# HKUST-Aerial-Robotics/Omni-swarm

Measured on AMD Instinct MI355X. Metric: keyframes/sec (4x fisheye 600x480) + p50 loop-match ms @ 100k-frame DB, higher is better.
Workload: dtype f16

## Files before the change

### omni-swarm_amd/csrc/config.h

```cpp
#pragma once
#include "common.h"

namespace omni {

enum CfgId {
    CFG_CONV_V1 = 0, CFG_RS_TRN, CFG_DET16, CFG_SP_SPARSE_DESC, CFG_SP_SPARSE_DA, CFG_SP_FUSED_CAND, CFG_SP_SPLIT_DB, CFG_SP_MASK_SKIP, CFG_SP_MASK_SKIP_SPLIT, CFG_SPLIT_FUSE1A, CFG_SPLIT_WINO,
    CFG_SPLIT_TRN, CFG_CONV_XCD, CFG_SP_PROFILE_MASK, CFG_PP_U8, CFG_PP_TRACE, CFG_PP_DBG, CFG_RS_TRACE, CFG_SPLIT_TRACE, CFG_SPLIT_DBG, CFG_WINO_TRACE, CFG_ROCTX,
    CFG_VLAD_BIG, CFG_VLAD_STEM_FUSE, CFG_VLAD_UNFUSED, CFG_VLAD_MFMA, CFG_VLAD_SBLOCK, CFG_VLAD_MBLOCK_PX, CFG_VLAD_MFMA_PX, CFG_VLAD_FC_MFMA, CFG_VLAD_MBLOCK_CPW,
    CFG_VLAD_SB_LDSPAD, CFG_VLAD_SB_PERSIST, CFG_VLAD_SB_TRACE, CFG_VLAD_SB_DBG, CFG_VLAD_MASK_SKIP,
    CFG_SCAN_ROWS_MIN, CFG_MQ_ROT, CFG_MQ_MIN, CFG_INDEX_MIRROR, CFG_INDEX_MIRROR_MIN_ROWS, CFG_INDEX_CERT_FAIL,
    CFG_GEOMETRY_THREADS, CFG_MESSAGE_THREADS, CFG_GEOMETRY_ASYNC, CFG_DETECTOR_ASYNC, CFG_PIPELINE_ONE_STREAM, CFG_PIPELINE_FIFO, CFG_PIPELINE_UNIT_PLAN,
    CFG_HW_QUEUES,
    CFG_RCCL_LIB,
    CFG_COUNT
};
enum CfgClass {
    CFG_VARIANT = 0,
    CFG_TUNING = 1,
    CFG_DEBUG = 2,
    CFG_TEST = 3,
    CFG_STRING = 4
};
struct CfgOption { const char* env; int def, lo, hi; int cls; const char* doc; };
extern const CfgOption kCfgOptions[CFG_COUNT];

struct Config {
    int v[CFG_COUNT];
    int operator[](CfgId i) const { return v[i]; }
};
int config_resolve(Config* out);
const Config& config_process();
int config_option_now(CfgId i);

}
```

### omni-swarm_amd/csrc/config.hip

```cpp
#include "config.h"

#include <atomic>
#include <cerrno>
#include <climits>
#include <cstdlib>

namespace omni {

const CfgOption kCfgOptions[CFG_COUNT] = {
    {"OMNI_CONV_V1", 0, 0, 3, CFG_VARIANT, "fp16 3x3 layers: 0 = production (conv1a fused into the ping-pong conv1b, register-stationary cin=128); 1 = generic kernel, 2 = persistent LDS-DMA kernel, "
                                           "3 = ping-pong without the conv1a fusion -- 1-3 exist only in the test build of the library (lib_test/)"},
    {"OMNI_RS_TRN", -1, -1, 1, CFG_VARIANT, "register-stationary kernel of the unpooled cin=128 fp16 layers: tile orientation, -1 = the one with fewer tiles, 0 = plain, 1 = transposed"},
    {"OMNI_DET16", 1, 0, 1, CFG_VARIANT, "detector head of the fp16 and OMNI_PREC_SPLIT paths on v_mfma_f32_32x32x16_f16 with split (hi, lo) operands (0: the exact-f32 MFMA kernel)"},
    {"OMNI_SP_SPARSE_DESC", 1, 0, 1, CFG_VARIANT, "convDb + descriptor norm only at the cells around the key points (0: dense descriptor map)"},
    {"OMNI_SP_SPARSE_DA", 1, 0, 1, CFG_VARIANT, "convDa only at those cells too (fp16 and OMNI_PREC_SPLIT; 0: dense convDa)"},
    {"OMNI_SP_FUSED_CAND", 1, 0, 1, CFG_VARIANT, "getKeyPoints' threshold inside the detector head's epilogue + window masks from the candidate list (0: sp_cand_kernel re-reads the heat map)"},
    {"OMNI_SP_SPLIT_DB", 1, 0, 1, CFG_VARIANT, "OMNI_PREC_SPLIT: convDb + descriptor norm at the key points' cells with split (hi, lo) operands on the fp16 matrix cores (0: exact-f32 MFMA convolution)"},
    {"OMNI_SP_MASK_SKIP", 1, 0, 1, CFG_VARIANT, "fp16: the tiles inside the constant region of the fisheye mask are left out of the tile walk (0: every tile)"},
    {"OMNI_SP_MASK_SKIP_SPLIT", 1, 0, 1, CFG_VARIANT, "the same for OMNI_PREC_SPLIT"},
    {"OMNI_SPLIT_FUSE1A", 1, 0, 1, CFG_VARIANT, "OMNI_PREC_SPLIT: conv1a built inside the conv1b kernel from the u8 image (0: separate exact-f32 conv1a pass)"},
    {"OMNI_SPLIT_WINO", 7, 0, 15, CFG_VARIANT, "OMNI_PREC_SPLIT: the cin = 64 layers as Winograd F(2x2,3x3) kernels with split operands (conv_wino.hip), bit 0 = conv1b (with the conv1a "
                                                "fusion), 1 = conv2a, 2 = conv2b, 3 = conv3a (off by default: same time as the direct kernel, profiles/r06g); 0: the direct kernels of conv_split.hip"},
    {"OMNI_SPLIT_TRN", -1, -1, 1, CFG_VARIANT, "OMNI_PREC_SPLIT cin=128 kernel: tile orientation, as OMNI_RS_TRN"},
    {"OMNI_CONV_XCD", 1, 0, 1, CFG_VARIANT, "persistent convolution kernels derive (cout group, tile walk) from an XCD-aware block id: the cout groups of a pixel tile and its neighbours "
                                           "share one L2 (0: plain blockIdx; process-wide, same results either way)"},
    {"OMNI_SP_PROFILE_MASK", 0, 0, 1, CFG_TUNING, "omni_sp_profile times the stages with the fisheye mask on (what the key-frame pipeline runs)"},
    {"OMNI_PP_U8", 1, 0, 1, CFG_VARIANT, "fp16 conv1a inside conv1b's kernel: matrix-core operands straight from the image bytes (0: through the 256-entry u8 -> (hi, lo) table in LDS)"},
    {"OMNI_PP_TRACE", 0, 0, 1, CFG_DEBUG, "s_memtime trace of the ping-pong conv kernel on stderr"},
    {"OMNI_PP_DBG", 0, 0, 255, CFG_DEBUG, "ping-pong conv kernel timing ablations (WRONG results)"},
    {"OMNI_RS_TRACE", 0, 0, 1, CFG_DEBUG, "s_memtime trace of the register-stationary kernel"},
    {"OMNI_SPLIT_TRACE", 0, 0, 1, CFG_DEBUG, "s_memtime trace of the split-precision kernel"},
    {"OMNI_SPLIT_DBG", 0, 0, 3, CFG_DEBUG, "split-precision kernel timing ablations: 1 = no stores, 2 = every DMA reads tile 0 (WRONG results)"},
    {"OMNI_WINO_TRACE", 0, 0, 1, CFG_DEBUG, "s_memtime trace of the Winograd split kernel"},
    {"OMNI_ROCTX", 0, 0, 1, CFG_DEBUG, "roctx ranges around upload / SuperPoint / MobileNetVLAD / post-processing / BF match / index add + search / exchange and the host loop's "
                                      "stages (rocprofv3 --marker-trace; the library is resolved by dlopen)"},
    {"OMNI_VLAD_BIG", 0, 0, 128, CFG_TUNING, "64 / 128: the 64- / 128-pixel tiles of the unfused block kernel (measured slower at 600x480)"},
    {"OMNI_VLAD_STEM_FUSE", 1, 0, 1, CFG_VARIANT, "stem + block 0 in one kernel (0: two kernels)"},
    {"OMNI_VLAD_UNFUSED", 0, 0, 1, CFG_VARIANT, "1: every block as expand / depthwise / project launches"},
    {"OMNI_VLAD_MFMA", 1, 0, 1, CFG_VARIANT, "late blocks' 1x1 convolutions on the matrix cores"},
    {"OMNI_VLAD_SBLOCK", 1, 0, 1, CFG_VARIANT, "fused split-fp16 block kernel (vlad_s.hip)"},
    {"OMNI_VLAD_MBLOCK_PX", 2048, 0, 1 << 24, CFG_TUNING, "fused matrix-core block kernel for blocks of at most this many input pixels per image (0 disables)"},
    {"OMNI_VLAD_MFMA_PX", 0, 0, 1 << 24, CFG_TUNING, "> 0: matrix-core 1x1 convolutions for blocks of at most this many input pixels per image (default 2048)"},
    {"OMNI_VLAD_FC_MFMA", 1, 0, 1, CFG_VARIANT, "the final FC on the matrix cores (0: VALU kernel)"},
    {"OMNI_VLAD_MBLOCK_CPW", 0, 0, 64, CFG_TUNING, "hidden-layer split of the matrix-core block kernel: chunks per workgroup (0 = no split; measured: does not pay)"},
    {"OMNI_VLAD_SB_LDSPAD", 0, 0, 160 * 1024, CFG_DEBUG, "extra LDS bytes per workgroup of the split block kernel (occupancy A/B)"},
    {"OMNI_VLAD_SB_PERSIST", 1, 0, 16, CFG_VARIANT, "split block kernel: 0 = one tile per workgroup, N >= 1 = N x (CUs x resident workgroups) persistent workgroups"},
    {"OMNI_VLAD_SB_TRACE", 0, 0, 1, CFG_DEBUG, "s_memtime trace of the split block kernel"},
    {"OMNI_VLAD_SB_DBG", 0, 0, 255, CFG_DEBUG, "split block kernel timing ablations (WRONG results)"},
    {"OMNI_VLAD_MASK_SKIP", 1, 0, 1, CFG_VARIANT, "fisheye-masked passes leave the tiles of the first blocks that lie in the constant region of the mask out of the tile walk "
                                                  "(bit-identical; 0: the dense pass)"},
    {"OMNI_SCAN_ROWS_MIN", 4, 1, 1 << 20, CFG_TUNING, "fp32 scan: from this many queries on, the rows-stationary kernel"},
    {"OMNI_MQ_ROT", 1, 0, 1, CFG_VARIANT, "matrix-core multi-query scan: rotated query fragments"},
    {"OMNI_MQ_MIN", 4, 0, 1 << 20, CFG_TUNING, "queries from which an fp16 shard is searched on the matrix cores (1 = always, 0 = never)"},
    {"OMNI_INDEX_MIRROR", 1, 0, 1, CFG_VARIANT, "fp32 index: fp16 mirror + certificate for batched searches (0: exact scans only)"},
    {"OMNI_INDEX_MIRROR_MIN_ROWS", 32768, 0, INT_MAX, CFG_TUNING, "the mirror is used from this many rows on"},
    {"OMNI_INDEX_CERT_FAIL", 0, 0, 1, CFG_TEST, "1: every certificate fails (exercises the exact fallback)"},
    {"OMNI_GEOMETRY_THREADS", -1, -1, 1024, CFG_TUNING, "threads of the geometric-verification pool (-1: min(16, cores / 2); 0: inline)"},
    {"OMNI_MESSAGE_THREADS", 3, 0, 64, CFG_TUNING, "helper threads that fill a unit's key-frame messages (key points, descriptors, lifted points: ~75 KB per image, first-touch page "
                                                  "faults included) next to the calling thread while the unit's detector step runs on the GPU (0: inline)"},
    {"OMNI_GEOMETRY_ASYNC", 1, 0, 1, CFG_VARIANT, "a micro-batch's geometry tasks run while the next unit is waited for (0: drained at once)"},
    {"OMNI_DETECTOR_ASYNC", 1, 0, 1, CFG_VARIANT, "a micro-batch's detector step (appends, searches) is enqueued and collected one unit later (0: the host waits for it on the spot)"},
    {"OMNI_PIPELINE_ONE_STREAM", 0, 0, 1, CFG_VARIANT, "a unit's MobileNetVLAD launches behind its SuperPoint launches on one stream (0: next to them on a second stream)"},
    {"OMNI_PIPELINE_FIFO", -1, -1, 2, CFG_VARIANT, "units in flight run oldest first: a unit's SuperPoint stream (1) / both its streams (2) start behind the convolution stack of the unit "
                                                   "enqueued before it; 0: the units' kernels take turns; -1: by measurement -- 1 for the fp32-class precisions, whose time is all "
                                                   "CU-filling convolutions (+2-4 %), and for an fp16 run() of no more units than lanes (all in flight at once: +13 % at 3 units), 0 for fp16 otherwise, whose small-grid "
                                                   "tails the next units' kernels fill (-5 % when chained)"},
    {"OMNI_PIPELINE_UNIT_PLAN", 1, 0, 2, CFG_VARIANT, "KeyframePipeline::run on host blocks, a run that is not a whole number of micro-batches: 1 = units of equal size (20 key frames = "
                                                       "7 + 7 + 6), 2 = the same behind half a unit, 0 = the blocks' own cut (8 + 8 + 4)"},
    {"OMNI_HW_QUEUES", 8, 0, 64, CFG_TUNING, "hardware queues asked of the HIP runtime when the library is loaded (GPU_MAX_HW_QUEUES, unless already set): the pipeline's five "
                                            "streams must not share one; 0 = the runtime's default of 4"},
    {"OMNI_RCCL_LIB", 0, 0, 0, CFG_STRING, "path of the RCCL library omni_shard dlopens (default: librccl.so next to torch, then the loader's search path)"},
};

static int parse_one(const CfgOption& o, int* out, bool* bad) {
    *out = o.def; *bad = false;
    if (o.cls == CFG_STRING) return 0;
    const char* e = getenv(o.env);
    if (!e || !e[0]) return 0;
    errno = 0;
    char* end = nullptr;
    const long v = strtol(e, &end, 10);
    if (errno || end == e || *end != '\0' || v < o.lo || v > o.hi) { *bad = true; return 0; }
    *out = (int)v;
    return 1;
}

int config_resolve(Config* out) {
    for (int i = 0; i < CFG_COUNT; ++i) {
        bool bad;
        parse_one(kCfgOptions[i], &out->v[i], &bad);
        OMNI_REQUIRE(!bad, OMNI_ERR_INVALID, "%s=%s: expected an integer in [%d, %d] (%s)", kCfgOptions[i].env, getenv(kCfgOptions[i].env), kCfgOptions[i].lo, kCfgOptions[i].hi,
                     kCfgOptions[i].doc);
    }
    return OMNI_OK;
}

static bool is_process_wide(int i) {
    switch (i) {
        case CFG_CONV_XCD: case CFG_INDEX_CERT_FAIL: case CFG_INDEX_MIRROR: case CFG_INDEX_MIRROR_MIN_ROWS: case CFG_MQ_ROT:
        case CFG_PP_DBG: case CFG_PP_TRACE: case CFG_RS_TRACE: case CFG_RS_TRN: case CFG_SCAN_ROWS_MIN: case CFG_SPLIT_DBG: case CFG_SPLIT_TRACE: case CFG_SPLIT_TRN: case CFG_WINO_TRACE: case CFG_ROCTX:
        case CFG_VLAD_BIG: case CFG_VLAD_SB_DBG: case CFG_VLAD_SB_LDSPAD: case CFG_VLAD_SB_TRACE:
            return true;
        default:
            return false;
    }
}
static std::atomic<bool> g_process_resolved{false};

int config_option_now(CfgId i) {
    int v; bool bad;
    parse_one(kCfgOptions[i], &v, &bad);
    return v;
}

const Config& config_process() {
    static const Config c = [] {
        g_process_resolved.store(true);
        Config q;
        for (int i = 0; i < CFG_COUNT; ++i) {
            bool bad;
            parse_one(kCfgOptions[i], &q.v[i], &bad);
            if (bad) fprintf(stderr, "libomni_hip: %s=%s ignored: expected an integer in [%d, %d]\n", kCfgOptions[i].env, getenv(kCfgOptions[i].env), kCfgOptions[i].lo, kCfgOptions[i].hi);
        }
        return q;
    }();
    return c;
}

}

extern "C" {

int omni_config_count(void) { return omni::CFG_COUNT; }

int omni_config_describe(int i, const char** env, int* def, int* lo, int* hi, int* cls, const char** doc) {
    OMNI_REQUIRE(i >= 0 && i < omni::CFG_COUNT, OMNI_ERR_INVALID, "omni_config_describe: option %d of %d", i, (int)omni::CFG_COUNT);
    const omni::CfgOption& o = omni::kCfgOptions[i];
    if (env) *env = o.env;
    if (def) *def = o.def;
    if (lo) *lo = o.lo;
    if (hi) *hi = o.hi;
    if (cls) *cls = o.cls;
    if (doc) *doc = o.doc;
    return OMNI_OK;
}

int omni_config_is_process_wide(int i) { return (i >= 0 && i < omni::CFG_COUNT && omni::is_process_wide(i)) ? 1 : 0; }

int omni_config_value(const char* env, int* value) {
    OMNI_REQUIRE(env && value, OMNI_ERR_INVALID, "null argument");
    omni::Config c;
    const int rc = omni::config_resolve(&c);
    if (rc) return rc;
    for (int i = 0; i < omni::CFG_COUNT; ++i)
        if (!strcmp(omni::kCfgOptions[i].env, env)) {
            *value = (omni::is_process_wide(i) && omni::g_process_resolved.load()) ? omni::config_process()[(omni::CfgId)i] : c.v[i];
            return OMNI_OK;
        }
    omni::set_error("omni_config_value: no option named %s", env);
    return OMNI_ERR_INVALID;
}

}
```

### omni-swarm_amd/csrc/conv.hip

```cpp
#include "config.h"
#include "conv.h"
#include <type_traits>

namespace omni {

typedef _Float16 half8_t __attribute__((ext_vector_type(8)));
typedef _Float16 half4_t __attribute__((ext_vector_type(4)));
typedef float floatx16 __attribute__((ext_vector_type(16)));
typedef float floatx4 __attribute__((ext_vector_type(4)));

template <typename T, int KG, int EPL>
static void pack_weights(const float* w, int cin, int cout, int ks, T* out) {
    const int taps = ks * ks, n_ct = cout / 64, n_ch = cin / 64;
    size_t o = 0;
    for (int ct = 0; ct < n_ct; ++ct)
        for (int ch = 0; ch < n_ch; ++ch)
            for (int tap = 0; tap < taps; ++tap)
                for (int kg = 0; kg < KG; ++kg)
                    for (int m = 0; m < 2; ++m)
                        for (int l = 0; l < 64; ++l)
                            for (int e = 0; e < EPL; ++e) {
                                const int co = ct * 64 + m * 32 + (l & 31);
                                const int ci = ch * 64 + kg * (64 / KG) + (l >> 5) * EPL + e;
                                const float v = w[((size_t)co * cin + ci) * taps + tap];
// ... 994 lines not shown
    hipLaunchKernelGGL(kfn, dim3(per_cg * n_cg), dim3(256), RS_SMEM, st, reinterpret_cast<const _Float16*>(a.in),
                       reinterpret_cast<_Float16*>(a.out), reinterpret_cast<const _Float16*>(a.w_packed), a.bias, a.H, a.W, a.cout, n_cg,
                       tiles_x, tiles_y, a.batch, a.relu ? 1 : 0, zero_page, want_trace ? trace_dev : nullptr, wk);
    OMNI_LAUNCH_CHECK();
    if (want_trace) {
        unsigned long long h[64];
        OMNI_HIP_TRY(hipMemcpyAsync(h, trace_dev, sizeof(h), hipMemcpyDeviceToHost, st));
        OMNI_HIP_TRY(hipStreamSynchronize(st));
        static int launches = 0;
        if (launches++ / 4 == 5)
            for (int k = 0; k < 8; ++k)
                fprintf(stderr, "rs trace H=%d W=%d cout=%d tile %llu (ty %llu tx %llu): issue %llu mfma %llu epilogue %llu wait %llu zerofix+barrier %llu | total %llu\n",
                        a.H, a.W, a.cout, h[k * 8 + 6], (h[k * 8 + 6] % (tiles_x * tiles_y)) / tiles_x, (h[k * 8 + 6] % (tiles_x * tiles_y)) % tiles_x,
                        h[k * 8 + 1] - h[k * 8], h[k * 8 + 2] - h[k * 8 + 1], h[k * 8 + 3] - h[k * 8 + 2], h[k * 8 + 4] - h[k * 8 + 3],
                        h[k * 8 + 5] - h[k * 8 + 4], h[k * 8 + 5] - h[k * 8]);
    }
    return OMNI_OK;
}

#define RS2_RING 3
template <int TH> struct Rs2Cfg {
    static constexpr int ITH = TH + 2, PIX = ITH * RS_ITW, NPIECES = (PIX * 16 + 63) / 64, PPW = (NPIECES + 3) / 4, BUF = NPIECES * 1024, NL = 3 * ITH * 8;
    static constexpr size_t smem() { return 2 * (size_t)BUF + 512; }
};
template <int L, int ITH>
__device__ __forceinline__ void rs2_read(uint32_t row_base , int n, int hh, half8_t& dst) {
    constexpr int kx = L / (ITH * 8), r = (L / 8) % ITH, kg = L % 8;
    constexpr int pc = r * RS_ITW + kx;
    const uint32_t addr = (row_base + pc * 256 + ((((pc + n) & 15) ^ hh) << 4)) ^ (kg << 5);
    asm volatile("ds_read_b128 %0, %1" : "=v"(dst) : "v"(addr));
}
template <int TH> constexpr int rs2_nmfma(int L) { const int r = (L / 8) % (TH + 2); int c = 0; for (int ky = 0; ky < 3; ++ky) if (r - ky >= 0 && r - ky < TH) ++c; return c; }
template <int TH> constexpr int rs2_count_before(int L, int want) { int c = 0; for (int l = 0; l < L; ++l) c += rs2_nmfma<TH>(l) == want ? 1 : 0; return c; }
template <int L, int TH, int NPARTS, int NDMA, typename Epi, typename Dma>
__device__ __forceinline__ void rs2_steps(uint32_t row_base, int n, int hh, const half8_t (&wreg)[72], floatx16 (&acc)[TH], half8_t (&fb)[RS2_RING], Epi&& epi, Dma&& dma) {
    constexpr int ITH = TH + 2, NL = 3 * ITH * 8;
    if constexpr (L < NL) {
        constexpr int kx = L / (ITH * 8), r = (L / 8) % ITH, kg = L % 8;
        constexpr int D = RS2_RING - 1;
        if constexpr (L + D < NL) rs2_read<L + D, ITH>(row_base, n, hh, fb[(L + D) % RS2_RING]);
        asm volatile("s_waitcnt lgkmcnt(%1)" : "+v"(fb[L % RS2_RING]) : "i"((L + D < NL) ? D : (NL - 1 - L)));
        __builtin_amdgcn_sched_barrier(0);
        constexpr int nm = rs2_nmfma<TH>(L);
        if constexpr (r >= 0 && r < TH) acc[r] = __builtin_amdgcn_mfma_f32_32x32x16_f16(wreg[(0 * 3 + kx) * 8 + kg], fb[L % RS2_RING], acc[r], 0, 0, 0);
        if constexpr (r - 1 >= 0 && r - 1 < TH) acc[r - 1] = __builtin_amdgcn_mfma_f32_32x32x16_f16(wreg[(1 * 3 + kx) * 8 + kg], fb[L % RS2_RING], acc[r - 1], 0, 0, 0);
        if constexpr (r - 2 >= 0 && r - 2 < TH) acc[r - 2] = __builtin_amdgcn_mfma_f32_32x32x16_f16(wreg[(2 * 3 + kx) * 8 + kg], fb[L % RS2_RING], acc[r - 2], 0, 0, 0);
        if constexpr (nm == 3) {
            constexpr int d = rs2_count_before<TH>(L, 3);
            if constexpr (d < NPARTS) {
                epi(std::integral_constant<int, d>{});
                __builtin_amdgcn_sched_group_barrier(0x008, 1, 0); __builtin_amdgcn_sched_group_barrier(0x002, 5, 0);
                __builtin_amdgcn_sched_group_barrier(0x008, 1, 0); __builtin_amdgcn_sched_group_barrier(0x002, 5, 0);
                __builtin_amdgcn_sched_group_barrier(0x008, 1, 0); __builtin_amdgcn_sched_group_barrier(0x002, 5, 0);
            }
        } else if constexpr (nm == 2) {
            constexpr int d = rs2_count_before<TH>(L, 2);
            if constexpr (d < NDMA) dma(std::integral_constant<int, d>{});
        }
        __builtin_amdgcn_sched_barrier(0);
        rs2_steps<L + 1, TH, NPARTS, NDMA>(row_base, n, hh, wreg, acc, fb, epi, dma);
    }
}

template <bool POOL, bool TRN = false>
__global__ void __launch_bounds__(256, 1)
conv3x3_c128_rs2_kernel(const _Float16* __restrict__ in, _Float16* __restrict__ out, const _Float16* __restrict__ wp,
                        const float* __restrict__ bias, int H, int W, int cout, int n_cg, int tiles_x, int tiles_y, int batch, int relu, TileWalk wk) {
    constexpr int TH = POOL ? 4 : 3;
    using C = Rs2Cfg<TH>;
    constexpr int ITH = C::ITH, PPW = C::PPW, NPIECES = C::NPIECES;
    static_assert(!TRN || !POOL, "transposed tiles: no pooling");
    extern __shared__ __attribute__((aligned(16))) char smem_raw[];
    const uint32_t lds0 = (uint32_t)(uintptr_t)(__attribute__((address_space(3))) char*)smem_raw;
    const int tid = threadIdx.x, lane = tid & 63;
    const int wave = __builtin_amdgcn_readfirstlane(tid >> 6);
    const int n = lane & 31, hh = lane >> 5;
    const int bid = xcd_block_id(wk.xcd);
    const int cg = bid % n_cg, wg = bid / n_cg, nwg = gridDim.x / n_cg;
    const int tiles_per_img = wk.act;
    const int total = batch * tiles_per_img;
    const int g32 = cg * 4 + wave;

    half8_t wreg[72];
    {
        const _Float16* wbase = wp + (int64_t)(g32 >> 1) * 2 * 9 * 4096 + (g32 & 1) * 512 + lane * 8;
#pragma unroll
        for (int s2 = 0; s2 < 72; ++s2) {
            const int tk = s2 >> 3, ch = (s2 >> 2) & 1, kg4 = s2 & 3;
            const int tap = TRN ? (tk % 3) * 3 + tk / 3 : tk;
            wreg[s2] = *reinterpret_cast<const half8_t*>(wbase + ((ch * 9 + tap) * 4 + kg4) * 1024);
        }
    }
    float* const bias_lds = reinterpret_cast<float*>(smem_raw + 2 * C::BUF);
    if (tid < 128) bias_lds[tid] = bias[cg * 128 + tid];

    auto tile_origin = [&](int t, int& b, int& ty0, int& tx0) {
        b = t / tiles_per_img;
        int ry, rx;
        tile_walk_rc<false>(wk, tiles_x, t - b * tiles_per_img, ry, rx);
        ty0 = ry * (TRN ? RS_TW : TH); tx0 = rx * (TRN ? TH : RS_TW);
    };
    uint32_t goff[PPW];
    uint32_t hx[(PPW + 4) / 5];
#pragma unroll
    for (int i = 0; i < (PPW + 4) / 5; ++i) hx[i] = 0;
#pragma unroll
    for (int j = 0; j < PPW; ++j) {
        int piece = wave * PPW + j;
        piece = piece < NPIECES ? piece : NPIECES - 1;
        const int idx = piece * 64 + lane;
        const int pix = idx >> 4, phys = idx & 15;
        const int iv = pix / RS_ITW, iu = pix - iv * RS_ITW;
        const int iy = TRN ? iu : iv, ix = TRN ? iv : iu;
        goff[j] = (uint32_t)((iy * W + ix) * 256 + ((phys ^ (pix & 15)) << 4));
        hx[j / 5] |= (uint32_t)(ix & 63) << (6 * (j % 5));
    }
    const uint32_t in_img_bytes = (uint32_t)H * W * 256u;
    struct Src { __amdgpu_buffer_rsrc_t r; uint32_t sorg; int x0; };
    auto source = [&](int t) -> Src {
        int b, ty0, tx0;
        tile_origin(t, b, ty0, tx0);
        Src s;
        s.r = __builtin_amdgcn_make_buffer_rsrc(const_cast<_Float16*>(in) + (int64_t)b * H * W * 128, 0, in_img_bytes, 0x00020000);
        s.x0 = tx0 - 1;
        s.sorg = (uint32_t)(((ty0 - 1) * W + s.x0) * 256);
        return s;
    };
    auto dma_piece = [&](const Src& s, int which, auto JC) {
        constexpr int j = decltype(JC)::value;
        int piece = wave * PPW + j;
        piece = piece < NPIECES ? piece : NPIECES - 1;
        const uint32_t x = (uint32_t)(s.x0 + (int)((hx[j / 5] >> (6 * (j % 5))) & 63u));
        const uint32_t voff = x < (uint32_t)W ? goff[j] + s.sorg : 0x80000000u;
#if __HIP_DEVICE_COMPILE__
        __builtin_amdgcn_raw_ptr_buffer_load_lds(s.r, (__attribute__((address_space(3))) void*)(smem_raw + which * C::BUF + piece * 1024), 16, voff, 0, 0, 0);
#else
        (void)s; (void)which; (void)piece; (void)voff;
#endif
    };
    int t = wg;
    if (t < total) {
        const Src s0 = source(t);
        spl2_for_each<0, PPW>([&](auto JC) { dma_piece(s0, 0, JC); });
    }
    asm volatile("s_waitcnt vmcnt(0)" ::: "memory");
    __syncthreads();
    float4 bs[4];
#pragma unroll
    for (int g = 0; g < 4; ++g) bs[g] = *reinterpret_cast<const float4*>(bias_lds + wave * 32 + 8 * g + 4 * hh);
    asm volatile("s_waitcnt lgkmcnt(0)" ::: "memory");
#pragma unroll
    for (int g = 0; g < 4; ++g) asm volatile("" : "+v"(bs[g].x), "+v"(bs[g].y), "+v"(bs[g].z), "+v"(bs[g].w));

    constexpr int NPF = POOL ? TH / 2 : TH;
    constexpr int NPARTS = NPF * 4;
    float pv[NPF][16];
    uint32_t poff[NPF];
#pragma unroll
    for (int f = 0; f < NPF; ++f) {
        poff[f] = 0x80000000u;
#pragma unroll
        for (int i = 0; i < 16; ++i) pv[f][i] = 0.f;
    }
    const uint32_t out_img_bytes = (uint32_t)((int64_t)(POOL ? (H >> 1) * (W >> 1) : H * W) * cout * 2);
    __amdgpu_buffer_rsrc_t oimg = __builtin_amdgcn_make_buffer_rsrc(out, 0, out_img_bytes, 0x00020000);
    uint32_t dq[2] = {0u, 0u};
    auto epi_part = [&](auto PC) {
        constexpr int P = decltype(PC)::value, f = P / 4, g = P % 4;
        float x[4];
#pragma unroll
        for (int e = 0; e < 4; ++e) {
            float v = pv[f][4 * g + e];
            if constexpr (POOL) v = vmax_med3(v, dpp_swap_pairs(v));
            x[e] = v;
        }
        const uint32_t d0 = pack_relu_f16<false>(x[0] + bs[g].x, x[1] + bs[g].y, 1), d1 = pack_relu_f16<false>(x[2] + bs[g].z, x[3] + bs[g].w, 1);
        if constexpr ((g & 1) == 0) { dq[0] = d0; dq[1] = d1; }
        else {
            const auto r0 = __builtin_amdgcn_permlane32_swap(dq[0], d0, false, false);
            const auto r1 = __builtin_amdgcn_permlane32_swap(dq[1], d1, false, false);
            typedef uint32_t u4_t __attribute__((ext_vector_type(4)));
            const u4_t dd = {r0[0], r1[0], r0[1], r1[1]};
            __builtin_amdgcn_raw_buffer_store_b128(dd, oimg, poff[f] + (uint32_t)((16 * (g >> 1) + 8 * hh) * 2), 0, 0);
        }
    };

    int cur = 0;
    for (; t < total; t += nwg, cur ^= 1) {
        const int tn = t + nwg;
        const Src sn = source(tn < total ? tn : t);
        const uint32_t row_base = lds0 + cur * C::BUF + n * 256;
        floatx16 acc[TH];
#pragma unroll
        for (int f = 0; f < TH; ++f)
#pragma unroll
            for (int i = 0; i < 16; ++i) acc[f][i] = 0.f;
        half8_t fb[RS2_RING];
        rs2_read<0, ITH>(row_base, n, hh, fb[0]);
        rs2_read<1, ITH>(row_base, n, hh, fb[1]);
        __builtin_amdgcn_sched_barrier(0);
        rs2_steps<0, TH, NPARTS, PPW>(row_base, n, hh, wreg, acc, fb, epi_part, [&](auto JC) { dma_piece(sn, cur ^ 1, JC); });

        int b, ty0, tx0;
        tile_origin(t, b, ty0, tx0);
        oimg = __builtin_amdgcn_make_buffer_rsrc(out + (int64_t)b * (out_img_bytes / 2), 0, out_img_bytes, 0x00020000);
        const int ox = tx0 + n;
        if constexpr (POOL) {
#pragma unroll
            for (int f2 = 0; f2 < TH / 2; ++f2) {
                const int oy = ty0 + 2 * f2;
#pragma unroll
                for (int i = 0; i < 16; ++i) pv[f2][i] = vmax_med3(acc[2 * f2][i], acc[2 * f2 + 1][i]);
                poff[f2] = ((oy < H) && (ox < W) && !(n & 1)) ? (uint32_t)((((oy >> 1) * (W >> 1) + (ox >> 1)) * cout + g32 * 32) * 2) : 0x80000000u;
            }
        } else {
#pragma unroll
            for (int f = 0; f < TH; ++f) {
                const int oy = TRN ? ty0 + n : ty0 + f, oxx = TRN ? tx0 + f : ox;
#pragma unroll
                for (int i = 0; i < 16; ++i) pv[f][i] = acc[f][i];
                poff[f] = ((oy < H) && (oxx < W)) ? (uint32_t)(((oy * W + oxx) * cout + g32 * 32) * 2) : 0x80000000u;
            }
        }
        asm volatile("s_waitcnt vmcnt(0)" ::: "memory");
        __syncthreads();
    }
    spl2_for_each<0, NPARTS>(epi_part);
}

static bool rs2_transposed(int H, int W) {
    static const int force = config_process()[CFG_RS_TRN];
    const int plain = cdiv(W, RS_TW) * cdiv(H, 3), trn = cdiv(W, 3) * cdiv(H, RS_TW);
    return force == 1 || (force < 0 && trn < plain);
}
template <bool POOL, bool TRN>
static int launch_conv_rs2(hipStream_t st, const ConvArgs& a, int n_cu) {
    constexpr int TH = POOL ? 4 : 3;
    OMNI_REQUIRE(a.relu, OMNI_ERR_INVALID, "conv_rs2: instantiated with the ReLU in its epilogue (every cin = 128 layer of the graph has one)");
    auto kfn = conv3x3_c128_rs2_kernel<POOL, TRN>;
    static DynSmemState smem_state;
    OMNI_HIP_TRY(ensure_dyn_smem(smem_state, (const void*)kfn, Rs2Cfg<TH>::smem()));
    const int tiles_x = cdiv(a.W, TRN ? TH : RS_TW), tiles_y = cdiv(a.H, TRN ? RS_TW : TH), n_cg = a.cout / 128;
    OMNI_REQUIRE((int64_t)a.H * a.W * 256 < (1ll << 31) && (int64_t)a.H * a.W * a.cout * 2 < (1ll << 31), OMNI_ERR_INVALID, "conv_rs2: image too large for 32-bit offsets");
    TileWalk wk;
    if (int rc = TRN ? tile_walk_plan(wk, "conv_rs2", tiles_x, tiles_y, 0, 0, 0, 0)
                     : tile_walk_plan(wk, "conv_rs2", tiles_x, tiles_y, a.skip_ty0, a.skip_ty1, a.skip_tx0, a.skip_tx1)) return rc;
    wk.xcd = config_process()[CFG_CONV_XCD];
    const int total = a.batch * wk.act;
    const int per_cg = tile_walk_grid(n_cu, n_cg, total);
    hipLaunchKernelGGL(kfn, dim3(per_cg * n_cg), dim3(256), Rs2Cfg<TH>::smem(), st, reinterpret_cast<const _Float16*>(a.in), reinterpret_cast<_Float16*>(a.out),
                       reinterpret_cast<const _Float16*>(a.w_packed), a.bias, a.H, a.W, a.cout, n_cg, tiles_x, tiles_y, a.batch, a.relu ? 1 : 0, wk);
    OMNI_LAUNCH_CHECK();
    return OMNI_OK;
}
int conv_rs_pool_tile_rows() { return RS_TH; }

template <int S, bool TRN>
__device__ __forceinline__ void spc_steps(uint32_t base, const half8_t (&wreg)[72], floatx16& acc, half8_t (&fb)[3]) {
    if constexpr (S < 72) {
        constexpr int o = S / 8, kg = S % 8, tap = TRN ? o : (o % 3) * 3 + o / 3;
        if constexpr (S + 2 < 72) {
            constexpr int o2 = (S + 2) / 8, kg2 = (S + 2) % 8, tap2 = TRN ? o2 : (o2 % 3) * 3 + o2 / 3;
            asm volatile("ds_read_b128 %0, %1 offset:%2" : "=v"(fb[(S + 2) % 3]) : "v"(base), "i"(tap2 * 256 + kg2 * 32));
        }
        asm volatile("s_waitcnt lgkmcnt(%1)" : "+v"(fb[S % 3]) : "i"((S + 2 < 72) ? 2 : (S + 1 < 72 ? 1 : 0)));
        __builtin_amdgcn_sched_barrier(0);
        acc = __builtin_amdgcn_mfma_f32_32x32x16_f16(wreg[tap * 8 + kg], fb[S % 3], acc, 0, 0, 0);
        __builtin_amdgcn_sched_barrier(0);
        spc_steps<S + 1, TRN>(base, wreg, acc, fb);
    }
}

#define SPC_CELL_BYTES 2320
#define SPC_BUF_BYTES (32 * SPC_CELL_BYTES)
#define SPC_SMEM (2 * SPC_BUF_BYTES)
template <bool TRN>
__global__ void __launch_bounds__(256, 1)
conv3x3_c128_sparse_kernel(const _Float16* __restrict__ in , const _Float16* __restrict__ wp, const float* __restrict__ bias,
                           int Hc, int Wc, int g32_first, int W, int H, int max_num, const float* __restrict__ kps_xy,
                           const int* __restrict__ n_kps, _Float16* __restrict__ out, int out_cstride, int tiles_per_img, int n_tiles,
                           const char* __restrict__ zero_page ) {
    extern __shared__ __attribute__((aligned(16))) char smem_raw[];
    const uint32_t lds0 = (uint32_t)(uintptr_t)(__attribute__((address_space(3))) char*)smem_raw;
    const int tid = threadIdx.x, lane = tid & 63;
    const int wave = __builtin_amdgcn_readfirstlane(tid >> 6);
    const int n = lane & 31, hh = lane >> 5;
    const int half = blockIdx.x & 1, wg = blockIdx.x >> 1, nwg = gridDim.x >> 1;
    const int g32 = g32_first + half * 4 + wave;
    half8_t wreg[72];
    {
        const _Float16* wbase = wp + (int64_t)(g32 >> 1) * 2 * 9 * 4096 + (g32 & 1) * 512 + lane * 8;
#pragma unroll
        for (int s2 = 0; s2 < 72; ++s2) {
            const int tap = s2 >> 3, ch = (s2 >> 2) & 1, kg4 = s2 & 3;
            wreg[s2] = *reinterpret_cast<const half8_t*>(wbase + ((ch * 9 + tap) * 4 + kg4) * 1024);
        }
    }
    float4 bs[4];
#pragma unroll
    for (int g = 0; g < 4; ++g) bs[g] = *reinterpret_cast<const float4*>(bias + g32 * 32 + 8 * g + 4 * hh);
    const float fW = (float)W, fH = (float)H, fWc = (float)Wc, fHc = (float)Hc;
    auto cell_of = [&](int t, int slot, int& b, int& kp, int& cx, int& cy) __attribute__((always_inline)) -> bool {
        b = t / tiles_per_img;
        kp = (t - b * tiles_per_img) * CSP_KP + (slot >> 2);
        cx = cy = -4;
        if (kp >= n_kps[b]) return false;
        const float kx = kps_xy[((int64_t)b * max_num + kp) * 2 + 0], ky = kps_xy[((int64_t)b * max_num + kp) * 2 + 1];
        const float gx = __fsub_rn(__fdiv_rn(__fmul_rn(2.0f, kx), fW), 1.0f);
        const float gy = __fsub_rn(__fdiv_rn(__fmul_rn(2.0f, ky), fH), 1.0f);
        const float ix = __fdiv_rn(__fsub_rn(__fmul_rn(__fadd_rn(gx, 1.0f), fWc), 1.0f), 2.0f);
        const float iy = __fdiv_rn(__fsub_rn(__fmul_rn(__fadd_rn(gy, 1.0f), fHc), 1.0f), 2.0f);
        cx = (int)floorf(ix) + (slot & 1); cy = (int)floorf(iy) + ((slot >> 1) & 1);
        return cx >= 0 && cx < Wc && cy >= 0 && cy < Hc;
    };
    const int gcell = tid >> 3, gpart = tid & 7;
    uint4 sa0, sb0, sa1, sb1, sa2, sb2, sa3, sb3, sa4, sb4, sa5, sb5, sa6, sb6, sa7, sb7, sa8, sb8;
    int fb, fkp, fcx, fcy; bool fok; const char* fimg;
#define SPC_FETCH_TAP(T)                                                                                                     \
    {                                                                                                                        \
        const int y = fcy + (T) / 3 - 1, x = fcx + (T) % 3 - 1;                                                              \
        const bool inside = fok && y >= 0 && y < Hc && x >= 0 && x < Wc;                                                     \
        const char* src = inside ? fimg + ((int64_t)y * Wc + x) * 256 + gpart * 16 : zero_page + (tid & 255) * 32;           \
        sa##T = *reinterpret_cast<const uint4*>(src);                                                                        \
        sb##T = *reinterpret_cast<const uint4*>(inside ? src + 128 : src + 16);                                              \
    }
#define SPC_FETCH(TILE)                                                                                                      \
    {                                                                                                                        \
        fok = cell_of((TILE), gcell, fb, fkp, fcx, fcy);                                                                     \
        fimg = reinterpret_cast<const char*>(in + (int64_t)fb * Hc * Wc * 128);                                              \
        SPC_FETCH_TAP(0) SPC_FETCH_TAP(1) SPC_FETCH_TAP(2) SPC_FETCH_TAP(3) SPC_FETCH_TAP(4) SPC_FETCH_TAP(5) SPC_FETCH_TAP(6) SPC_FETCH_TAP(7) SPC_FETCH_TAP(8) \
    }
#define SPC_PARK_TAP(T) *reinterpret_cast<uint4*>(pdst + (T) * 256) = sa##T; *reinterpret_cast<uint4*>(pdst + (T) * 256 + 128) = sb##T;
#define SPC_PARK(WHICH)                                                                                                      \
    {                                                                                                                        \
        char* pdst = smem_raw + (WHICH) * SPC_BUF_BYTES + gcell * SPC_CELL_BYTES + gpart * 16;                               \
        SPC_PARK_TAP(0) SPC_PARK_TAP(1) SPC_PARK_TAP(2) SPC_PARK_TAP(3) SPC_PARK_TAP(4) SPC_PARK_TAP(5) SPC_PARK_TAP(6) SPC_PARK_TAP(7) SPC_PARK_TAP(8) \
    }
    int t = wg;
    if (t < n_tiles) { SPC_FETCH(t) SPC_PARK(0) }
    __syncthreads();
    int cur = 0;
    for (; t < n_tiles; t += nwg, cur ^= 1) {
        const int tn = t + nwg;
        if (tn < n_tiles) SPC_FETCH(tn)
        floatx16 acc;
#pragma unroll
        for (int r = 0; r < 16; ++r) acc[r] = 0.f;
        {
            const uint32_t base = lds0 + cur * SPC_BUF_BYTES + n * SPC_CELL_BYTES + hh * 16;
            half8_t fb[3];
            asm volatile("s_waitcnt lgkmcnt(0)" ::: "memory");
            asm volatile("ds_read_b128 %0, %1 offset:%2" : "=v"(fb[0]) : "v"(base), "i"(0));
            asm volatile("ds_read_b128 %0, %1 offset:%2" : "=v"(fb[1]) : "v"(base), "i"(32));
            __builtin_amdgcn_sched_barrier(0);
            spc_steps<0, TRN>(base, wreg, acc, fb);
        }
        {
            int b, kp, cx, cy;
            const bool ok = cell_of(t, n, b, kp, cx, cy);
            if (ok) {
                _Float16* op = out + (((int64_t)b * max_num + kp) * 4 + (n & 3)) * out_cstride + (g32 - g32_first) * 32 + 4 * hh;
#pragma unroll
                for (int g = 0; g < 4; ++g) {
                    const uint32_t d0 = pack_relu_f16<false>(acc[4 * g + 0] + bs[g].x, acc[4 * g + 1] + bs[g].y, 1);
                    const uint32_t d1 = pack_relu_f16<false>(acc[4 * g + 2] + bs[g].z, acc[4 * g + 3] + bs[g].w, 1);
                    *reinterpret_cast<uint2*>(op + 8 * g) = make_uint2(d0, d1);
                }
            }
        }
        if (tn < n_tiles) SPC_PARK(cur ^ 1)
        __syncthreads();
    }
#undef SPC_FETCH_TAP
#undef SPC_FETCH
#undef SPC_PARK_TAP
#undef SPC_PARK
}

int conv_c128_sparse(hipStream_t st, const omni_ctx* ctx, const void* in_f16, const void* w_packed, const float* bias, int Hc, int Wc, int g32_first,
                     int W, int H, int max_num, const float* kps_xy, const int* n_kps, void* out_f16, int out_cstride, int batch) {
    const int tiles_per_img = cdiv(max_num, CSP_KP), n_tiles = tiles_per_img * batch;
    const int cus = ctx->prop.multiProcessorCount > 0 ? ctx->prop.multiProcessorCount : 256;
    int pairs = cus / 2;
    if (pairs > n_tiles) pairs = n_tiles;
    if (pairs < 1) pairs = 1;
    const bool trn = rs2_transposed(Hc, Wc);
    OMNI_REQUIRE(ctx->zero_page, OMNI_ERR_INVALID, "conv_c128_sparse: the context has no zero block");
    auto launch = [&](auto kfn) -> int {
        static DynSmemState attr;
        OMNI_HIP_TRY(ensure_dyn_smem(attr, (const void*)kfn, SPC_SMEM));
        hipLaunchKernelGGL(kfn, dim3(2 * pairs), dim3(256), SPC_SMEM, st, (const _Float16*)in_f16, (const _Float16*)w_packed, bias, Hc, Wc, g32_first, W, H,
                           max_num, kps_xy, n_kps, (_Float16*)out_f16, out_cstride, tiles_per_img, n_tiles, (const char*)ctx->zero_page);
        OMNI_LAUNCH_CHECK();
        return OMNI_OK;
    };
    return trn ? launch(conv3x3_c128_sparse_kernel<true>) : launch(conv3x3_c128_sparse_kernel<false>);
}

template <typename T, int KS, bool POOL>
static int launch_conv(hipStream_t st, const ConvArgs& a) {
    const size_t smem = conv_smem_bytes<T, KS>();
    auto kfn = conv_mfma_kernel<T, KS, POOL>;
    OMNI_HIP_TRY(hipFuncSetAttribute((const void*)kfn, hipFuncAttributeMaxDynamicSharedMemorySize, (int)smem));
    dim3 grid(cdiv(a.W, CONV_TW) * cdiv(a.H, CONV_TH), a.cout / CONV_COUT_TILE, a.batch);
    hipLaunchKernelGGL(kfn, grid, dim3(256), smem, st, reinterpret_cast<const T*>(a.in), a.out, reinterpret_cast<const T*>(a.w_packed),
                       a.bias, a.H, a.W, a.cin, a.cout, a.relu ? 1 : 0, a.out_f32 ? 1 : 0, a.in_cstride > 0 ? a.in_cstride : a.cin);
    OMNI_LAUNCH_CHECK();
    return OMNI_OK;
}

int conv1ab_fused(hipStream_t st, const ConvArgs& a, const uint8_t* gray, int gstride, int fisheye_mask, const _Float16* w1a_frag,
                  const float* bias1a, const uint32_t* lut_hl) {
    OMNI_REQUIRE(a.cin == 64 && a.cout % 64 == 0 && a.ksize == 3 && a.pool && a.n_cu > 0, OMNI_ERR_INVALID, "conv1ab_fused: bad layer shape");
    OMNI_REQUIRE(gstride % 4 == 0 && ((uintptr_t)gray & 3) == 0 && (int64_t)a.batch * a.H * gstride < (1ll << 31), OMNI_ERR_INVALID,
                 "conv1ab_fused: image rows must be 4-byte aligned (stride %d)", gstride);
    Fuse1aArgs fz;
    fz.gray = gray; fz.gstride = gstride;
    omni_fisheye_mask_rows(a.H, fisheye_mask, &fz.mask_r0, &fz.mask_r1);
    fz.w1a_frag = w1a_frag; fz.bias1a = bias1a; fz.lut_hl = lut_hl; fz.trace = nullptr;
    static const bool want_trace = config_process()[CFG_PP_TRACE] != 0;
    static unsigned long long* trace_dev = nullptr;
    if (want_trace) {
        if (!trace_dev) OMNI_HIP_TRY(hipMalloc((void**)&trace_dev, 64 * 8));
        OMNI_HIP_TRY(hipMemsetAsync(trace_dev, 0, 64 * 8, st));
        fz.trace = trace_dev;
    }
    static const int dbg = config_process()[CFG_PP_DBG];
    const int rc = launch_conv_pp_abl<true, 0, true>(st, a, a.n_cu, dbg, fz);
    if (want_trace && rc == OMNI_OK) {
        unsigned long long h[64];
        OMNI_HIP_TRY(hipMemcpyAsync(h, trace_dev, sizeof(h), hipMemcpyDeviceToHost, st));
        OMNI_HIP_TRY(hipStreamSynchronize(st));
        static int printed = 0;
        if (printed++ == 20)
            for (int p = 2; p < 6; ++p)
                fprintf(stderr, "pp trace phase %d: service start %llu issue +%llu epilogue +%llu build +%llu (operands ready +%llu, first fragment +%llu) | mfma loop %llu cycles (start +%lld vs service start)\n", p,
                        h[p * 8], h[p * 8 + 1] - h[p * 8], h[p * 8 + 2] - h[p * 8 + 1], h[p * 8 + 3] - h[p * 8 + 2], h[p * 8 + 6] - h[p * 8 + 2], h[p * 8 + 7] - h[p * 8 + 6],
                        h[p * 8 + 5] - h[p * 8 + 4], (long long)(h[p * 8 + 4] - h[p * 8]));
    }
    return rc;
}

static inline uint16_t f2h_bits(float v) { const __half h = __float2half_rn(v); uint16_t u; memcpy(&u, &h, 2); return u; }
static inline float h2f(uint16_t u) { __half h; memcpy(&h, &u, 2); return __half2float(h); }
void conv1a_pack_split_weights(const float* w, const float* bias, uint16_t* frag ) {
    for (int j = 0; j < 2; ++j)
        for (int m = 0; m < 2; ++m)
            for (int l = 0; l < 64; ++l)
                for (int e = 0; e < 8; ++e) {
                    const int co = m * 32 + (l & 31), hh = l >> 5;
                    auto hi = [&](int t) { return f2h_bits(w[co * 9 + t]); };
                    auto lo = [&](int t) { return f2h_bits(w[co * 9 + t] - h2f(f2h_bits(w[co * 9 + t]))); };
                    uint16_t v = 0;
                    if (j == 0) v = hi((hh ? 5 : 0) + e / 2);
                    else if (hh == 0) v = e < 2 ? hi(4) : (e < 7 ? lo(e - 2) : 0);
                    else v = e < 4 ? lo(5 + e) : (e == 4 ? f2h_bits(bias[co]) : (e == 5 ? f2h_bits(bias[co] - h2f(f2h_bits(bias[co]))) : 0));
                    frag[((j * 2 + m) * 64 + l) * 8 + e] = v;
                }
}
void conv1a_pack_u8_weights(const float* w, const float* bias, uint16_t* frag ) {
    for (int m = 0; m < 2; ++m)
        for (int l = 0; l < 64; ++l) {
            const int co = m * 32 + (l & 31), hh = l >> 5;
            uint16_t Wh[9], Wl[9];
            double sum = 0.0;
            for (int t = 0; t < 9; ++t) {
                const float W = (float)((double)w[co * 9 + t] * 256.0 / 255.0);
                Wh[t] = f2h_bits(W); Wl[t] = f2h_bits(W - h2f(Wh[t]));
                sum += (double)h2f(Wh[t]) + (double)h2f(Wl[t]);
            }
            const float b = (float)((double)bias[co] - 4.0 * sum);
            const uint16_t bh = f2h_bits(b), bl = f2h_bits(b - h2f(bh));
            for (int j = 0; j < 2; ++j)
                for (int e = 0; e < 8; ++e) {
                    uint16_t v = 0;
                    if (j == 0) { const int t = (hh ? 5 : 0) + e / 2; v = (e & 1) ? Wl[t] : Wh[t]; }
                    else if (hh == 0) v = e == 0 ? Wh[4] : (e == 1 ? Wl[4] : 0);
                    else v = e == 0 ? bh : (e == 1 ? bl : 0);
                    frag[((j * 2 + m) * 64 + l) * 8 + e] = v;
                }
        }
}
void conv1a_make_split_lut(uint32_t* lut ) {
    for (int i = 0; i < 256; ++i) {
        const volatile float alpha = (float)(1.0 / 255.0);
        const float x = (float)i * alpha;
        const uint16_t hi = f2h_bits(x);
        lut[i] = (uint32_t)hi | ((uint32_t)f2h_bits(x - h2f(hi)) << 16);
    }
}

int conv_mfma(hipStream_t st, int precision, const ConvArgs& a) {
    OMNI_REQUIRE(a.cin % 64 == 0 && a.cout % 64 == 0, OMNI_ERR_INVALID, "conv_mfma: cin=%d cout=%d must be multiples of 64", a.cin, a.cout);
    OMNI_REQUIRE(a.ksize == 1 || a.ksize == 3, OMNI_ERR_INVALID, "conv_mfma: ksize=%d", a.ksize);
    OMNI_REQUIRE(!a.pool || (a.H % 2 == 0 && a.W % 2 == 0), OMNI_ERR_INVALID, "pooling needs even H, W");
    OMNI_REQUIRE(!(a.pool && a.ksize == 1), OMNI_ERR_INVALID, "1x1 + pool not instantiated");
    if (precision == OMNI_PREC_F16 && a.ksize == 3 && a.cin == 64 && !a.out_f32 && (a.in_cstride == 0 || a.in_cstride == 64) && a.n_cu > 0 && a.zero_page &&
        a.variant != 1) {
#ifdef OMNI_TEST_VARIANTS
        if (a.variant == 2) return a.pool ? launch_conv_c64<true>(st, a, a.n_cu) : launch_conv_c64<false>(st, a, a.n_cu);
#endif
        return a.pool ? launch_conv_pp<true>(st, a, a.n_cu) : launch_conv_pp<false>(st, a, a.n_cu);
    }
    if (precision == OMNI_PREC_F16 && a.ksize == 3 && a.cin == 128 && a.cout % 128 == 0 && !a.out_f32 && (a.in_cstride == 0 || a.in_cstride == 128) &&
        a.n_cu > 0 && a.zero_page && a.variant == 0 && (!a.pool || a.H % 2 == 0))
    {
        if (a.pool) return launch_conv_rs(st, a, a.n_cu);
        return rs2_transposed(a.H, a.W) ? launch_conv_rs2<false, true>(st, a, a.n_cu) : launch_conv_rs2<false, false>(st, a, a.n_cu);
    }
    if (precision == OMNI_PREC_F16) {
#ifdef OMNI_TEST_VARIANTS
        if (a.ksize == 3) return a.pool ? launch_conv<_Float16, 3, true>(st, a) : launch_conv<_Float16, 3, false>(st, a);
#else
        OMNI_REQUIRE(a.ksize != 3, OMNI_ERR_INVALID, "conv_mfma: no production fp16 kernel for a 3x3 layer with cin=%d cout=%d in_cstride=%d (the generic one is only built into the test library)",
                     a.cin, a.cout, a.in_cstride);
#endif
        return launch_conv<_Float16, 1, false>(st, a);
    } else {
        if (a.ksize == 3) return a.pool ? launch_conv<float, 3, true>(st, a) : launch_conv<float, 3, false>(st, a);
        return launch_conv<float, 1, false>(st, a);
    }
}

template <typename T>
__global__ void __launch_bounds__(256)
conv1a_kernel(const uint8_t* __restrict__ gray, int stride, int H, int W, int mask_row0, int mask_row1,
              const float* __restrict__ w, const float* __restrict__ bias, const float* __restrict__ lut, T* __restrict__ out) {
    __shared__ float tile[10][36];
    __shared__ float wsm[9][64];
    __shared__ float bsm[64];
    __shared__ float lsm[256];
    const int tid = threadIdx.x;
    const int tiles_x = (W + 31) / 32;
    const int ty0 = (blockIdx.x / tiles_x) * 8, tx0 = (blockIdx.x % tiles_x) * 32;
    const int b = blockIdx.y;
    const uint8_t* g = gray + (int64_t)b * stride * H;
    lsm[tid] = lut[tid];
    for (int i = tid; i < 576; i += 256) { const int co = i / 9, tap = i - co * 9; wsm[tap][co] = w[i]; }
    if (tid < 64) bsm[tid] = bias[tid];
    __syncthreads();
    for (int i = tid; i < 340; i += 256) {
        const int iy = i / 34, ix = i - iy * 34;
        const int gy = ty0 - 1 + iy, gx = tx0 - 1 + ix;
        float v = 0.f;
        if (gy >= 0 && gy < H && gx >= 0 && gx < W && !(gy >= mask_row0 && gy < mask_row1)) v = lsm[g[(int64_t)gy * stride + gx]];
        tile[iy][ix] = v;
    }
    __syncthreads();
#pragma unroll 1
    for (int it = 0; it < 8; ++it) {
        const int wi = tid + it * 256;
        const int pix = wi >> 3, cg = wi & 7;
        const int py = pix >> 5, px = pix & 31;
        float acc[8];
#pragma unroll
        for (int j = 0; j < 8; ++j) acc[j] = bsm[cg * 8 + j];
#pragma unroll
        for (int tap = 0; tap < 9; ++tap) {
            const float v = tile[py + tap / 3][px + tap % 3];
#pragma unroll
            for (int j = 0; j < 8; ++j) acc[j] = fmaf(v, wsm[tap][cg * 8 + j], acc[j]);
        }
        const int gy = ty0 + py, gx = tx0 + px;
        if (gy < H && gx < W) {
            T* o = out + (((int64_t)b * H + gy) * W + gx) * 64 + cg * 8;
            if constexpr (sizeof(T) == 4) {
                *reinterpret_cast<float4*>(o) = make_float4(fmaxf(acc[0], 0.f), fmaxf(acc[1], 0.f), fmaxf(acc[2], 0.f), fmaxf(acc[3], 0.f));
                *reinterpret_cast<float4*>(o + 4) = make_float4(fmaxf(acc[4], 0.f), fmaxf(acc[5], 0.f), fmaxf(acc[6], 0.f), fmaxf(acc[7], 0.f));
            } else {
                half8_t h;
#pragma unroll
                for (int j = 0; j < 8; ++j) h[j] = (_Float16)fmaxf(acc[j], 0.f);
                *reinterpret_cast<half8_t*>(o) = h;
            }
        }
    }
}

int conv1a_direct(hipStream_t st, int precision, const uint8_t* gray, int stride, int batch, int H, int W, int fisheye_mask,
                  const float* w, const float* bias, const float* lut, void* out) {
    int r0, r1;
    omni_fisheye_mask_rows(H, fisheye_mask, &r0, &r1);
    dim3 grid(cdiv(W, 32) * cdiv(H, 8), batch);
    if (precision == OMNI_PREC_F16)
        hipLaunchKernelGGL(conv1a_kernel<_Float16>, grid, dim3(256), 0, st, gray, stride, H, W, r0, r1, w, bias, lut, (_Float16*)out);
    else
        hipLaunchKernelGGL(conv1a_kernel<float>, grid, dim3(256), 0, st, gray, stride, H, W, r0, r1, w, bias, lut, (float*)out);
    OMNI_LAUNCH_CHECK();
    return OMNI_OK;
}

__device__ __forceinline__ float wave_sum_f(float v) {
#pragma unroll
    for (int off = 32; off > 0; off >>= 1) v += __shfl_xor(v, off, 64);
    return v;
}
__device__ __forceinline__ float wave_max_f(float v) {
#pragma unroll
    for (int off = 32; off > 0; off >>= 1) v = fmaxf(v, __shfl_xor(v, off, 64));
    return v;
}

#define DET_THREADS 512
#define DET_WAVES (DET_THREADS / 64)
#define DET_CPW 4
template <typename T>
__global__ void __launch_bounds__(DET_THREADS)
detector_head_kernel(const T* __restrict__ in, int in_stride, int in_off, int n_cells, int Hc, int Wc,
                     const float* __restrict__ wT, const float* __restrict__ bias, float* __restrict__ semi) {
    extern __shared__ __attribute__((aligned(16))) char smem_raw[];
    float* wTs = reinterpret_cast<float*>(smem_raw);
    float* xs = wTs + 256 * 65;
    const int tid = threadIdx.x, lane = tid & 63, wave = tid >> 6;
    for (int i = tid; i < 256 * 65; i += DET_THREADS) wTs[i] = wT[i];
    const float my_bias = bias[lane];
    const float dust_bias = bias[64];
    __syncthreads();
    float* x = xs + wave * DET_CPW * 256;
    for (int base = blockIdx.x * DET_WAVES * DET_CPW; base < n_cells; base += gridDim.x * DET_WAVES * DET_CPW) {
        const int cell0 = base + wave * DET_CPW;
#pragma unroll
        for (int c = 0; c < DET_CPW; ++c) {
            const int cell = cell0 + c;
            float4 v = make_float4(0.f, 0.f, 0.f, 0.f);
            if (cell < n_cells) {
                const T* ip = in + (int64_t)cell * in_stride + in_off + lane * 4;
                if constexpr (sizeof(T) == 4) {
                    v = *reinterpret_cast<const float4*>(ip);
                } else {
                    const half4_t h = *reinterpret_cast<const half4_t*>(ip);
                    v = make_float4((float)h[0], (float)h[1], (float)h[2], (float)h[3]);
                }
            }
            *reinterpret_cast<float4*>(x + c * 256 + lane * 4) = v;
        }
        __syncthreads();
        float acc[DET_CPW], dpart[DET_CPW];
#pragma unroll
        for (int c = 0; c < DET_CPW; ++c) { acc[c] = my_bias; dpart[c] = 0.f; }
        for (int k = 0; k < 256; k += 4) {
            const float w0 = wTs[(k + 0) * 65 + lane], w1 = wTs[(k + 1) * 65 + lane];
            const float w2 = wTs[(k + 2) * 65 + lane], w3 = wTs[(k + 3) * 65 + lane];
#pragma unroll
            for (int c = 0; c < DET_CPW; ++c) {
                const float4 xv = *reinterpret_cast<const float4*>(x + c * 256 + k);
                acc[c] = fmaf(xv.x, w0, acc[c]);
                acc[c] = fmaf(xv.y, w1, acc[c]);
                acc[c] = fmaf(xv.z, w2, acc[c]);
                acc[c] = fmaf(xv.w, w3, acc[c]);
            }
        }
#pragma unroll
        for (int j = 0; j < 4; ++j) {
            const float wd = wTs[(lane * 4 + j) * 65 + 64];
#pragma unroll
            for (int c = 0; c < DET_CPW; ++c) dpart[c] = fmaf(x[c * 256 + lane * 4 + j], wd, dpart[c]);
        }
#pragma unroll
        for (int c = 0; c < DET_CPW; ++c) {
            const int cell = cell0 + c;
// ... 714 lines not shown
```

Measured before the change: 2700.

## Route fp16 pooled cin=128 conv to pipelined rs2 kernel with in-register 2x2 pool

The pooled conv3b layer now runs by default on the v5 pipelined register-stationary kernel (rs2) instead of the v4 kernel. The v4 path stays behind a debug flag for A/B and bit-identity checks. The rs2 pool epilogue is reworked: vertical max runs across accumulator rows, a DPP pair swap handles the horizontal max, and odd and even lanes each store a different pooled row, so only one partial-store set is held instead of TH/2. The mask-skip tile rows are rescaled from the v4 tile height to rs2's, which may skip fewer tiles.

After: 2737, median of 6. 1.4% higher.

```diff
diff --git a/omni-swarm_amd/csrc/config.h b/omni-swarm_amd/csrc/config.h
--- a/omni-swarm_amd/csrc/config.h
+++ b/omni-swarm_amd/csrc/config.h
@@ -5,7 +5,7 @@
 
 enum CfgId {
     CFG_CONV_V1 = 0, CFG_RS_TRN, CFG_DET16, CFG_SP_SPARSE_DESC, CFG_SP_SPARSE_DA, CFG_SP_FUSED_CAND, CFG_SP_SPLIT_DB, CFG_SP_MASK_SKIP, CFG_SP_MASK_SKIP_SPLIT, CFG_SPLIT_FUSE1A, CFG_SPLIT_WINO,
-    CFG_SPLIT_TRN, CFG_CONV_XCD, CFG_SP_PROFILE_MASK, CFG_PP_U8, CFG_PP_TRACE, CFG_PP_DBG, CFG_RS_TRACE, CFG_SPLIT_TRACE, CFG_SPLIT_DBG, CFG_WINO_TRACE, CFG_ROCTX,
+    CFG_SPLIT_TRN, CFG_CONV_XCD, CFG_SP_PROFILE_MASK, CFG_PP_U8, CFG_PP_TRACE, CFG_PP_DBG, CFG_RS_TRACE, CFG_RS_POOL_V4, CFG_SPLIT_TRACE, CFG_SPLIT_DBG, CFG_WINO_TRACE, CFG_ROCTX,
     CFG_VLAD_BIG, CFG_VLAD_STEM_FUSE, CFG_VLAD_UNFUSED, CFG_VLAD_MFMA, CFG_VLAD_SBLOCK, CFG_VLAD_MBLOCK_PX, CFG_VLAD_MFMA_PX, CFG_VLAD_FC_MFMA, CFG_VLAD_MBLOCK_CPW,
     CFG_VLAD_SB_LDSPAD, CFG_VLAD_SB_PERSIST, CFG_VLAD_SB_TRACE, CFG_VLAD_SB_DBG, CFG_VLAD_MASK_SKIP,
     CFG_SCAN_ROWS_MIN, CFG_MQ_ROT, CFG_MQ_MIN, CFG_INDEX_MIRROR, CFG_INDEX_MIRROR_MIN_ROWS, CFG_INDEX_CERT_FAIL,
diff --git a/omni-swarm_amd/csrc/config.hip b/omni-swarm_amd/csrc/config.hip
--- a/omni-swarm_amd/csrc/config.hip
+++ b/omni-swarm_amd/csrc/config.hip
@@ -29,6 +29,8 @@
     {"OMNI_PP_TRACE", 0, 0, 1, CFG_DEBUG, "s_memtime trace of the ping-pong conv kernel on stderr"},
     {"OMNI_PP_DBG", 0, 0, 255, CFG_DEBUG, "ping-pong conv kernel timing ablations (WRONG results)"},
     {"OMNI_RS_TRACE", 0, 0, 1, CFG_DEBUG, "s_memtime trace of the register-stationary kernel"},
+    {"OMNI_RS_POOL_V4", 0, 0, 1, CFG_DEBUG, "fp16 conv3b+pool on the v4 register-stationary kernel instead of v5's pipelined pooled form (A/B and bit-identity reference; "
+                                            "OMNI_RS_TRACE traces v4 only)"},
     {"OMNI_SPLIT_TRACE", 0, 0, 1, CFG_DEBUG, "s_memtime trace of the split-precision kernel"},
     {"OMNI_SPLIT_DBG", 0, 0, 3, CFG_DEBUG, "split-precision kernel timing ablations: 1 = no stores, 2 = every DMA reads tile 0 (WRONG results)"},
     {"OMNI_WINO_TRACE", 0, 0, 1, CFG_DEBUG, "s_memtime trace of the Winograd split kernel"},
@@ -98,7 +100,7 @@
 static bool is_process_wide(int i) {
     switch (i) {
         case CFG_CONV_XCD: case CFG_INDEX_CERT_FAIL: case CFG_INDEX_MIRROR: case CFG_INDEX_MIRROR_MIN_ROWS: case CFG_MQ_ROT:
-        case CFG_PP_DBG: case CFG_PP_TRACE: case CFG_RS_TRACE: case CFG_RS_TRN: case CFG_SCAN_ROWS_MIN: case CFG_SPLIT_DBG: case CFG_SPLIT_TRACE: case CFG_SPLIT_TRN: case CFG_WINO_TRACE: case CFG_ROCTX:
+        case CFG_PP_DBG: case CFG_PP_TRACE: case CFG_RS_TRACE: case CFG_RS_POOL_V4: case CFG_RS_TRN: case CFG_SCAN_ROWS_MIN: case CFG_SPLIT_DBG: case CFG_SPLIT_TRACE: case CFG_SPLIT_TRN: case CFG_WINO_TRACE: case CFG_ROCTX:
         case CFG_VLAD_BIG: case CFG_VLAD_SB_DBG: case CFG_VLAD_SB_LDSPAD: case CFG_VLAD_SB_TRACE:
             return true;
         default:
diff --git a/omni-swarm_amd/csrc/conv.hip b/omni-swarm_amd/csrc/conv.hip
--- a/omni-swarm_amd/csrc/conv.hip
+++ b/omni-swarm_amd/csrc/conv.hip
@@ -1170,7 +1170,7 @@
 #pragma unroll
     for (int g = 0; g < 4; ++g) asm volatile("" : "+v"(bs[g].x), "+v"(bs[g].y), "+v"(bs[g].z), "+v"(bs[g].w));
 
-    constexpr int NPF = POOL ? TH / 2 : TH;
+    constexpr int NPF = POOL ? 1 : TH;
     constexpr int NPARTS = NPF * 4;
     float pv[NPF][16];
     uint32_t poff[NPF];
@@ -1187,11 +1187,7 @@
         constexpr int P = decltype(PC)::value, f = P / 4, g = P % 4;
         float x[4];
 #pragma unroll
-        for (int e = 0; e < 4; ++e) {
-            float v = pv[f][4 * g + e];
-            if constexpr (POOL) v = vmax_med3(v, dpp_swap_pairs(v));
-            x[e] = v;
-        }
+        for (int e = 0; e < 4; ++e) x[e] = pv[f][4 * g + e];
         const uint32_t d0 = pack_relu_f16<false>(x[0] + bs[g].x, x[1] + bs[g].y, 1), d1 = pack_relu_f16<false>(x[2] + bs[g].z, x[3] + bs[g].w, 1);
         if constexpr ((g & 1) == 0) { dq[0] = d0; dq[1] = d1; }
         else {
@@ -1222,19 +1218,19 @@
         int b, ty0, tx0;
         tile_origin(t, b, ty0, tx0);
         oimg = __builtin_amdgcn_make_buffer_rsrc(out + (int64_t)b * (out_img_bytes / 2), 0, out_img_bytes, 0x00020000);
-        const int ox = tx0 + n;
         if constexpr (POOL) {
-#pragma unroll
-            for (int f2 = 0; f2 < TH / 2; ++f2) {
-                const int oy = ty0 + 2 * f2;
-#pragma unroll
-                for (int i = 0; i < 16; ++i) pv[f2][i] = vmax_med3(acc[2 * f2][i], acc[2 * f2 + 1][i]);
-                poff[f2] = ((oy < H) && (ox < W) && !(n & 1)) ? (uint32_t)((((oy >> 1) * (W >> 1) + (ox >> 1)) * cout + g32 * 32) * 2) : 0x80000000u;
-            }
+            const bool odd = n & 1;
+#pragma unroll
+            for (int i = 0; i < 16; ++i) {
+                const float q0 = vmax_med3(acc[0][i], acc[1][i]), q1 = vmax_med3(acc[2][i], acc[3][i]);
+                pv[0][i] = vmax_med3(odd ? q1 : q0, dpp_swap_pairs(odd ? q0 : q1));
+            }
+            const int oy = ty0 + (odd ? 2 : 0), px = tx0 + (n & ~1);
+            poff[0] = ((oy < H) && (px < W)) ? (uint32_t)((((oy >> 1) * (W >> 1) + (px >> 1)) * cout + g32 * 32) * 2) : 0x80000000u;
         } else {
 #pragma unroll
             for (int f = 0; f < TH; ++f) {
-                const int oy = TRN ? ty0 + n : ty0 + f, oxx = TRN ? tx0 + f : ox;
+                const int oy = TRN ? ty0 + n : ty0 + f, oxx = TRN ? tx0 + f : tx0 + n;
 #pragma unroll
                 for (int i = 0; i < 16; ++i) pv[f][i] = acc[f][i];
                 poff[f] = ((oy < H) && (oxx < W)) ? (uint32_t)(((oy * W + oxx) * cout + g32 * 32) * 2) : 0x80000000u;
@@ -1261,8 +1257,9 @@
     const int tiles_x = cdiv(a.W, TRN ? TH : RS_TW), tiles_y = cdiv(a.H, TRN ? RS_TW : TH), n_cg = a.cout / 128;
     OMNI_REQUIRE((int64_t)a.H * a.W * 256 < (1ll << 31) && (int64_t)a.H * a.W * a.cout * 2 < (1ll << 31), OMNI_ERR_INVALID, "conv_rs2: image too large for 32-bit offsets");
     TileWalk wk;
+    const int sy0 = POOL ? cdiv(a.skip_ty0 * RS_TH, TH) : a.skip_ty0, sy1 = POOL ? a.skip_ty1 * RS_TH / TH : a.skip_ty1;
     if (int rc = TRN ? tile_walk_plan(wk, "conv_rs2", tiles_x, tiles_y, 0, 0, 0, 0)
-                     : tile_walk_plan(wk, "conv_rs2", tiles_x, tiles_y, a.skip_ty0, a.skip_ty1, a.skip_tx0, a.skip_tx1)) return rc;
+                     : tile_walk_plan(wk, "conv_rs2", tiles_x, tiles_y, sy0, sy1, a.skip_tx0, a.skip_tx1)) return rc;
     wk.xcd = config_process()[CFG_CONV_XCD];
     const int total = a.batch * wk.act;
     const int per_cg = tile_walk_grid(n_cu, n_cg, total);
@@ -1523,7 +1520,8 @@
     if (precision == OMNI_PREC_F16 && a.ksize == 3 && a.cin == 128 && a.cout % 128 == 0 && !a.out_f32 && (a.in_cstride == 0 || a.in_cstride == 128) &&
         a.n_cu > 0 && a.zero_page && a.variant == 0 && (!a.pool || a.H % 2 == 0))
     {
-        if (a.pool) return launch_conv_rs(st, a, a.n_cu);
+        static const bool pool_v4 = config_process()[CFG_RS_POOL_V4] != 0;
+        if (a.pool) return pool_v4 ? launch_conv_rs(st, a, a.n_cu) : launch_conv_rs2<true, false>(st, a, a.n_cu);
         return rs2_transposed(a.H, a.W) ? launch_conv_rs2<false, true>(st, a, a.n_cu) : launch_conv_rs2<false, false>(st, a, a.n_cu);
     }
     if (precision == OMNI_PREC_F16) {
```
